# pennneutrinos/chroma

Measured on AMD Instinct MI355X. Metric: photons/sec (propagate_hit), higher is better.
Workload: dtype f32

## Files before the change

### chroma_amd/csrc/chroma_hip.hip

```cpp
#include <math.h>
#include <stdio.h>
#include <stdlib.h>
#include <string.h>
#include <algorithm>

#ifndef CHROMA_EXPERIMENTAL
#define CHROMA_EXPERIMENTAL 0
#endif
#ifndef CHROMA_HYBRID_RENDER
#define CHROMA_HYBRID_RENDER 1
#endif
#include "chroma_internal.h"
#include "propagate_device.h"

#include "kernel_propagate_fused.h"

#include "kernel_step_control.h"

#include "kernels_raycast_crosscheck.h"

#include "kernel_raycast_quad.h"

#include "kernel_raycast_pair.h"

// ... 175 lines not shown
    std::vector<Slab> slabs;
};

static void tracks_release(chroma_ctx *ctx, chroma_tracks *tr)
{
    if (!tr) return;
    for (const chroma_tracks::Slab &s : tr->slabs) chroma_free(ctx, s.rows);
    chroma_free(ctx, tr->rows0);
    chroma_free(ctx, tr->offsets);
    delete tr;
}

namespace { struct PropagateCall; }
static int propagate_order(PropagateCall &call, uint32_t **d_order);

namespace {
struct PropagateCall {
    const CallScope &scope; CallState &cs;
    chroma_ctx *ctx; chroma_geometry *geom;
    CallPlan plan;
    PhotonView pv; chroma_rng rng; chroma_propagate_options opt;
    uint64_t nphotons; uint32_t ncopies;
    uint32_t *in_q, *out_q;
    float4 *work_in, *work_out;
    float4 *rays, *rays_next;
    float4 *final_rec;
    uint32_t final_epoch;
    HitsOut ho;
    bool finalize;
    chroma_propagate_stats acc;
    long long n_upper;
    bool finalized;
    chroma_tracks *tracks;

    hipEvent_t *events(int step) const { return opt.time_kernels ? cs.step_events.data() + EV_PER_STEP * step : nullptr; }

    int load_working()
    {
        const unsigned blocks = (unsigned)std::min<uint64_t>((nphotons + PHYS_BLOCK - 1) / PHYS_BLOCK, (uint64_t)ctx->physics_blocks);
        int rc = scope.clear_words(W_PACKET_USE, W_PACKET_END - W_PACKET_USE); if (rc) return rc;
        uint32_t *d_order = nullptr;
        rc = propagate_order(*this, &d_order); if (rc) return rc;
        hipLaunchKernelGGL(k_load_working, dim3(blocks), dim3(PHYS_BLOCK), 0, ctx->stream, geom->view, pv, in_q, work_in,
                           (uint64_t)nphotons, ncopies, (uint32_t)(nphotons / ncopies), plan.chain ? rays : nullptr,
                           plan.packet == 2 ? cs.d_words + W_PACKET_COHERENT : nullptr, (const uint32_t *)d_order, plan.cast == Cast::LITERAL ? 1 : 0);
        if (d_order) { chroma_free(ctx, d_order); acc.reordered += nphotons; }
#if CHROMA_EXPERIMENTAL
        if (plan.packet)
            hipLaunchKernelGGL(k_packet_decide, dim3(1), dim3(1), 0, ctx->stream, cs.d_words + W_PACKET_COHERENT, cs.d_words + W_PACKET_USE,
                               (uint64_t)nphotons, plan.packet);
#endif
        HIP_TRY(hipGetLastError());
        return CHROMA_OK;
    }

    void launch_step_begin(uint32_t first_n)
    {
        hipLaunchKernelGGL(k_step_begin, dim3(1), dim3(1), 0, ctx->stream, in_q, out_q, cs.d_step,
                           tracks ? 0u : opt.use_weights ? 0xFFFFFFFFu : (uint32_t)(PROP_BLOCK * 16 * 8), first_n);
    }

    void launch_physics(int scatter_first, int fixup)
    {
        StepState *st = cs.d_step;
        float4 *chained = plan.chain ? rays_next : nullptr;
        const bool plain = geom->view.plain_optics != 0;
        bool deal = false;
#if PHYS_DEAL
        deal = plain && !final_rec;
#endif
        const int pb = deal ? PHYS_DEAL_BLOCK : PHYS_BLOCK_OF(!plain);
        unsigned blocks = (unsigned)std::min<long long>((n_upper + pb - 1) / pb, std::max<long long>(1, (long long)ctx->physics_blocks * PHYS_BLOCK / pb));
        if (fixup == 1 && plain) blocks = std::max(std::min(blocks, 64u), blocks / 8);
        DeviceCounters *pc = plan.counting ? cs.d_counters : nullptr;
#if PHYS_DEAL
        if (deal) {
            hipLaunchKernelGGL(k_physics_deal, dim3(blocks), dim3(PHYS_DEAL_BLOCK), 0, ctx->stream, geom->view, pv, st, work_in, out_q, work_out,
                               cs.hit_triangle, cs.hit_distance, rng.seed, rng.photon_id_base, opt.use_weights, scatter_first,
                               cs.retry_list, fixup, pc, chained);
            return;
        }
#endif
        const int literal_rays = fixup == 2 ? 1 : 0;
        with_bool(!plain, [&](auto FULL) {
            hipLaunchKernelGGL((k_physics<FULL>), dim3(blocks), dim3(PHYS_BLOCK_OF(FULL)), 0, ctx->stream, geom->view, pv, st, work_in, out_q,
                               work_out, cs.hit_triangle, cs.hit_distance, rng.seed, rng.photon_id_base, opt.use_weights, scatter_first,
                               cs.retry_list, fixup, pc, chained, final_rec, final_epoch, literal_rays);
        });
    }

    int launch_split_step(int scatter_first, hipEvent_t *ev, uint32_t first_n, bool packet)
    {
        if (n_upper <= 0) return CHROMA_OK;
        StepState *st = cs.d_step;
        const Cast cast = plan.cast;
        const bool exact = cast == Cast::LITERAL || cast == Cast::LITERAL_LANE;
        const dim3 block(PROP_BLOCK);
        auto record = [&](int slot) { return ev ? hipEventRecord(ev[slot], ctx->stream) : hipSuccess; };
        const unsigned rblocks = (unsigned)std::min<long long>((n_upper + PROP_BLOCK - 1) / PROP_BLOCK, 8 * 256);
        auto retry = [&](auto C) {
            hipLaunchKernelGGL((k_raycast_retry<C>), dim3(rblocks), block, 0, ctx->stream, geom->view, rays, st, cs.hit_triangle,
                               cs.hit_distance, cs.retry_list, cs.d_counters);
        };
        launch_step_begin(first_n);
        HIP_TRY(record(EV_STEP_BEGIN));
        if (!plan.chain) {
            unsigned sblocks = (unsigned)std::min<long long>((n_upper + 255) / 256, (long long)ctx->physics_blocks * 4);
            hipLaunchKernelGGL(k_ray_setup, dim3(sblocks), dim3(256), 0, ctx->stream, geom->view, work_in, st, rays,
                               cs.hit_triangle, cs.hit_distance, cs.retry_list, &st->retry, cast == Cast::LITERAL ? 1 : 0);
        }
        HIP_TRY(record(EV_PACKET_BEGIN));
        const uint32_t *skip_quad = nullptr;
#if CHROMA_EXPERIMENTAL
        if (packet) {
            skip_quad = cs.d_words + W_PACKET_USE;
            const unsigned pwaves = (unsigned)std::min<long long>((n_upper + WAVE - 1) / WAVE, (long long)ctx->waves[(int)Cast::QUAD]);
            with_bool(plan.counting, [&](auto C) {
                hipLaunchKernelGGL((k_raycast_packet<C>), dim3(pwaves), block, 0, ctx->stream, geom->view, rays, st, cs.hit_triangle,
                                   cs.hit_distance, cs.retry_list, cs.d_counters, cs.d_words + W_PACKET_USE);
            });
        }
#else
        (void)packet;
#endif
        HIP_TRY(record(EV_CAST_BEGIN));
        const dim3 grid(cast_waves(ctx, cast, n_upper));
        const int chained = plan.chain ? 1 : 0;
        with_bool(plan.counting, [&](auto C) {
            switch (cast) {
            case Cast::PAIR:
                hipLaunchKernelGGL((k_raycast_pair<C>), grid, block, 0, ctx->stream, geom->view, rays, 0, st, cs.hit_triangle,
                                   cs.hit_distance, cs.retry_list, cs.coop_spill, cs.d_counters, ctx->coop_chunk);
                break;
            case Cast::QUAD:
                hipLaunchKernelGGL((k_raycast_quad<C>), grid, block, 0, ctx->stream, geom->view, rays, 0, st, cs.hit_triangle,
                                   cs.hit_distance, cs.retry_list, cs.coop_spill, cs.d_counters, ctx->coop_chunk, chained, skip_quad,
                                   ctx->claim_static);
                break;
            case Cast::COOP:
                hipLaunchKernelGGL((k_raycast_coop<C>), grid, block, 0, ctx->stream, geom->view, rays, 0, st, cs.hit_triangle,
                                   cs.hit_distance, cs.retry_list, cs.coop_spill, cs.d_counters, ctx->coop_chunk);
                break;
            case Cast::WIDE:
                hipLaunchKernelGGL((k_raycast_wide<C>), grid, block, 0, ctx->stream, geom->view, rays, 0, st, cs.hit_triangle,
                                   cs.hit_distance, cs.retry_list, cs.wide_spill, cs.d_counters, ctx->ray_chunk);
                break;
            case Cast::PERSISTENT:
                hipLaunchKernelGGL((k_raycast_persistent<C>), grid, block, 0, ctx->stream, geom->view, rays, 0, st, cs.hit_triangle,
                                   cs.hit_distance, cs.retry_list, cs.d_counters);
                break;
            case Cast::LITERAL:
                hipLaunchKernelGGL((k_raycast_literal<C>), grid, block, 0, ctx->stream, geom->view, rays, st, cs.hit_triangle,
                                   cs.hit_distance, cs.coop_spill, cs.d_counters, ctx->coop_chunk, chained, cs.retry_list,
                                   ctx->claim_static);
                retry(C);
                break;
            case Cast::LITERAL_LANE:
                hipLaunchKernelGGL((k_raycast_retry<C, true>), grid, block, 0, ctx->stream, geom->view, rays, st, cs.hit_triangle,
                                   cs.hit_distance, cs.retry_list, cs.d_counters);
                break;
            }
        });
        HIP_TRY(record(EV_CAST_END));
        launch_physics(scatter_first, exact ? 2 : 0);
        HIP_TRY(record(EV_PHYSICS_END));
        if (!exact) {
            with_bool(plan.counting, retry);
            launch_physics(scatter_first, 1);
        }
        HIP_TRY(record(EV_STEP_END));
// ... 756 lines not shown
```

### chroma_amd/csrc/chroma_internal.h

```cpp
#pragma once
#include <hip/hip_runtime.h>
#include <stdint.h>
#include <array>
#include <map>
#include <mutex>
#include <type_traits>
#include <unordered_map>
#include <vector>

#include <rccl/rccl.h>

#include "device_common.h"

#define CHROMA_LOCAL __attribute__((visibility("hidden")))

CHROMA_LOCAL int set_error(int code, const char *fmt, ...);

#define HIP_TRY(expr)                                                                          \
    do {                                                                                       \
        hipError_t e_ = (expr);                                                                \
        if (e_ != hipSuccess)                                                                  \
            return set_error((int)e_, "%s failed: %s (%s:%d)", #expr, hipGetErrorString(e_), __FILE__, __LINE__); \
    } while (0)

struct CallState {
    uint32_t *queue_a = nullptr, *queue_b = nullptr;
    size_t queue_capacity = 0;
    int32_t *hit_triangle = nullptr;
    float *hit_distance = nullptr;
    uint32_t *retry_list = nullptr;
    float4 *rays = nullptr;
    float4 *rays_b = nullptr;
    float4 *work_a = nullptr, *work_b = nullptr;
    float4 *final_rec = nullptr; size_t final_capacity = 0; uint32_t final_epoch = 0;
    DeviceCounters *d_counters = nullptr;
    uint32_t *d_words = nullptr;
    uint32_t *h_words = nullptr;
    StepState *d_step = nullptr;
    uint32_t *h_step = nullptr;
    std::vector<hipEvent_t> step_events;
    uint2 *wide_spill = nullptr;
    uint2 *coop_spill = nullptr;
    hipEvent_t ev_start = nullptr, ev_stop = nullptr, ev_mid = nullptr;
    hipStream_t aux_stream = nullptr;
    void *call_scratch = nullptr; size_t call_scratch_bytes = 0;
    bool particles_have = false; const void *particles_block = nullptr; size_t particles_block_bytes = 0;
    chroma_particle_arrays particles_run = {}; int32_t particles_max_steps = 0;
    hipEvent_t ev_fork = nullptr, ev_join = nullptr;
    int counting = 0;
    int tail_mode = CHROMA_TAIL_COOP;
    int autosort_mode = 0;
    int packet_mode = 0;
    int walk = CHROMA_WALK_QUAD;
};

struct chroma_ctx {
    int device;
    hipStream_t stream;
    int physics_blocks = 256 * 8;
    int waves[CHROMA_WALK_LITERAL_LANE + 1] = {};
    int ray_chunk = 256, coop_chunk = 64;
    int claim_static = 5 | 8 << 4;
    ncclComm_t comm = nullptr;
    int comm_nranks = 1, comm_rank = 0;
    uint32_t *gather_buf = nullptr;
    size_t gather_capacity = 0;
    struct PoolBlock { void *ptr; hipEvent_t ev; };
    std::mutex pool_mu;
    std::multimap<size_t, PoolBlock> pool;
    std::unordered_map<void *, size_t> live;
    std::vector<hipEvent_t> pool_events;
    size_t pool_bytes = 0, pool_limit = 0;
    uint64_t pool_hits = 0, pool_misses = 0;
    hipStream_t copy_stream = nullptr;
    std::mutex stage_mu;
    static constexpr int STAGE_N = 3;
    static constexpr size_t STAGE_BYTES = 64u << 20;
    void *stage[STAGE_N] = {nullptr, nullptr, nullptr};
    hipEvent_t stage_ev[STAGE_N] = {nullptr, nullptr, nullptr};
    std::mutex stage_down_mu;
    void *stage_down[STAGE_N] = {nullptr, nullptr, nullptr};
    hipEvent_t stage_down_ev[STAGE_N] = {nullptr, nullptr, nullptr};
private:
    friend class CallScope;
    std::mutex call_mu;
    CallState call_state;
};

struct chroma_geometry {
    chroma_ctx *ctx;
    GeoView view;
    std::vector<void *> allocations;
    void *d_vertices = nullptr, *d_triangles = nullptr, *d_material_codes = nullptr, *d_colors = nullptr;
    void *d_nodes_api = nullptr;
    size_t nvertices = 0, ntriangles = 0, nnodes = 0, nwide = 0, nrecords = 0;
    uint32_t stack_need = 0, wide_depth = 0, wide_stack_need = 0;
    size_t device_bytes = 0;
};

enum ScratchWord {
    W_HIT_COUNT = 0,
    W_SURVIVORS = 1,
    W_ABORT = 2,
    W_RESULT_END = 3,
    W_PACKET_USE = 4,
    W_PACKET_COHERENT = 5, W_PACKET_WAVES = 6, W_PACKET_END = 7,
    W_ORDER_PROBE = 8, W_ORDER_PROBE_END = 11,
    SCRATCH_WORDS = 16
};

class CallScope {
public:
    explicit CallScope(chroma_ctx *c) : ctx(c), lock_(c->call_mu) {}
    CallScope(const CallScope &) = delete;
    CallScope &operator=(const CallScope &) = delete;
    CallState &state() const { return ctx->call_state; }

    int clear_words(ScratchWord first, int count = 1) const
    {
        HIP_TRY(hipMemsetAsync(state().d_words + first, 0, count * sizeof(uint32_t), ctx->stream));
        return CHROMA_OK;
    }
    int clear_results() const { return clear_words(W_HIT_COUNT, W_RESULT_END - W_HIT_COUNT); }
    int read_words(ScratchWord first, int count = 1) const { return read_back(first, state().d_words + first, count); }
    int read_results() const { return read_words(W_HIT_COUNT, W_RESULT_END - W_HIT_COUNT); }
    uint32_t word(ScratchWord slot) const { return state().h_words[slot]; }
    int read_word(ScratchWord slot, uint32_t *out) const
    {
        const int rc = read_words(slot);
        *out = word(slot);
        return rc;
    }
    int read_survivors(const uint32_t *d_queue, long long *n) const
    {
        const int rc = read_back(W_SURVIVORS, d_queue, 1);
        *n = (long long)word(W_SURVIVORS) - 1;
        return rc;
    }

    chroma_ctx *const ctx;
private:
    int read_back(ScratchWord slot, const uint32_t *d_src, int count) const
    {
        HIP_TRY(hipMemcpyAsync(state().h_words + slot, d_src, count * sizeof(uint32_t), hipMemcpyDeviceToHost, ctx->stream));
        HIP_TRY(hipStreamSynchronize(ctx->stream));
        return CHROMA_OK;
    }
    std::lock_guard<std::mutex> lock_;
};

struct QueueBuffer { void **ptr; size_t bytes; };
static inline std::array<QueueBuffer, 9> queue_buffers(CallState &c)
{
    return {{{(void **)&c.queue_a, sizeof(uint32_t)}, {(void **)&c.queue_b, sizeof(uint32_t)},
             {(void **)&c.hit_triangle, sizeof(int32_t)}, {(void **)&c.hit_distance, sizeof(float)},
             {(void **)&c.retry_list, sizeof(uint32_t)}, {(void **)&c.rays, 4 * sizeof(float4)}, {(void **)&c.rays_b, 4 * sizeof(float4)},
             {(void **)&c.work_a, 4 * sizeof(float4)}, {(void **)&c.work_b, 4 * sizeof(float4)}}};
}

CHROMA_LOCAL hipError_t ctx_malloc(chroma_ctx *ctx, void **ptr, size_t bytes);

static int grow_call_scratch(const CallScope &scope, size_t need, bool *grew = nullptr)
{
    CallState &cs = scope.state();
    if (grew) *grew = false;
    if (cs.call_scratch_bytes >= need) return CHROMA_OK;
    HIP_TRY(hipStreamSynchronize(scope.ctx->stream));
    if (cs.call_scratch) { HIP_TRY(hipFree(cs.call_scratch)); cs.call_scratch = nullptr; cs.call_scratch_bytes = 0; }
    HIP_TRY(ctx_malloc(scope.ctx, &cs.call_scratch, need));
    cs.call_scratch_bytes = need;
    if (grew) *grew = true;
    return CHROMA_OK;
}

// ... 62 lines not shown
```

### chroma_amd/csrc/device_common.h

```cpp
#pragma once

#include <hip/hip_runtime.h>
#include <stdint.h>

#define CM_FN __host__ __device__ static inline
#include "../../include/chroma_math.h"
#include "../../include/chroma_hip.h"

#define WAVE 64

typedef float f32x2 __attribute__((ext_vector_type(2)));

struct v3 { float x, y, z; };
__device__ inline v3 mk3(float x, float y, float z) { return v3{x, y, z}; }
__device__ inline v3 operator-(v3 a) { return mk3(-a.x, -a.y, -a.z); }
__device__ inline v3 operator+(v3 a, v3 b) { return mk3(a.x + b.x, a.y + b.y, a.z + b.z); }
__device__ inline v3 operator-(v3 a, v3 b) { return mk3(a.x - b.x, a.y - b.y, a.z - b.z); }
__device__ inline v3 operator*(v3 a, float c) { return mk3(a.x * c, a.y * c, a.z * c); }
__device__ inline v3 operator*(float c, v3 a) { return mk3(c * a.x, c * a.y, c * a.z); }
__device__ inline v3 operator/(v3 a, float c) { return mk3(a.x / c, a.y / c, a.z / c); }
__device__ inline v3 operator/(v3 a, v3 b) { return mk3(a.x / b.x, a.y / b.y, a.z / b.z); }
__device__ inline v3 operator/(float c, v3 a) { return mk3(c / a.x, c / a.y, c / a.z); }
__device__ inline float dot(v3 a, v3 b) { return a.x * b.x + a.y * b.y + a.z * b.z; }
__device__ inline v3 cross(v3 a, v3 b)
{ return mk3(a.y * b.z - a.z * b.y, a.z * b.x - a.x * b.z, a.x * b.y - a.y * b.x); }
__device__ inline float norm(v3 a) { return cm_sqrtf(dot(a, a)); }
__device__ inline v3 normalize(v3 a) { return a / norm(a); }

__device__ inline v3 load3(const float *p, size_t i) { return mk3(p[3 * i], p[3 * i + 1], p[3 * i + 2]); }
__device__ inline void store3(float *p, size_t i, v3 v) { p[3 * i] = v.x; p[3 * i + 1] = v.y; p[3 * i + 2] = v.z; }

__device__ inline float interp_table(float x, int n, const float *xp, const float *fp)
{
    int lower = 0;
    int upper = n - 1;
    if (x <= xp[lower]) return fp[lower];
    if (x >= xp[upper]) return fp[upper];
    while (lower < upper - 1) {
        int half = (lower + upper) / 2;
        if (x < xp[half]) upper = half; else lower = half;
    }
    float df = fp[upper] - fp[lower];
    float dx = xp[upper] - xp[lower];
    return fp[lower] + df * (x - xp[lower]) / dx;
}

struct SurfaceInfo { uint32_t model; uint32_t transmissive; float thickness; int32_t dichroic_index; };

#ifndef TRI_STRIDE
#define TRI_STRIDE 3
#endif
struct GeoView {
    const uint4  *nodes;
    const uint4  *wnodes;
    const float4 *tri;
    const float4 *tri_isect;
    const uint4  *tri_phys;
    const uint32_t *tri_to_dev, *dev_to_tri;
    const float *mat_refractive_index, *mat_absorption_length, *mat_scattering_length;
    const uint32_t *mat_num_comp, *mat_comp_offset;
    const float *comp_reemission_prob, *comp_reemission_wvl_cdf, *comp_absorption_length, *comp_reemission_time_cdf;
    const float *surf_detect, *surf_absorb, *surf_reemit, *surf_reflect_diffuse, *surf_reflect_specular,
                *surf_eta, *surf_k, *surf_reemission_cdf;
    const SurfaceInfo *surf_info;
    const uint32_t *dichroic_nangles, *dichroic_offset;
    const float *dichroic_angles, *dichroic_reflect, *dichroic_transmit;
    const uint32_t *solid_id_map;
    const int32_t  *solid_id_to_channel_index;
    float world_origin[3];
    float world_scale;
    float suspect_margin;
    float slab_grow;
    uint32_t wavelength_n; float wavelength_start, wavelength_step;
    uint32_t time_n;       float time_start, time_step;
    uint32_t nnodes, ntriangles, nsolids, nchannels, nwide;
    uint32_t plain_optics;
};

struct TriPhys { v3 normal; uint32_t code, id, bx, by, bz; };
__device__ inline TriPhys load_tri_phys(const GeoView &g, size_t record)
{
    const uint4 *r = g.tri_phys + 2 * record;
    const uint4 a = r[0], b = r[1];
    return TriPhys{mk3(__uint_as_float(a.x), __uint_as_float(a.y), __uint_as_float(a.z)), a.w, b.x, b.y, b.z, b.w};
}

struct PhotonView {
    float *pos, *dir, *pol, *wavelengths, *t;
    uint32_t *flags; int32_t *last_hit_triangles; float *weights; uint32_t *evidx; uint32_t *rng_counters;
};

struct DeviceCounters {
    unsigned long long photon_steps, nodes_visited, triangles_tested, stack_overflows;
    unsigned long long stack_spills;
    unsigned long long packet_rays, packet_nodes, packet_tris;
};

struct StepState {
    uint32_t n;
    uint32_t renorm;
    uint32_t in_tail;
    uint32_t launches;
    uint32_t work;
    uint32_t retry;
    uint32_t pad[2];
};

__device__ inline int hit_channel(const GeoView &g, uint32_t history, int triangle_id, uint32_t detection_state)
{
    if (!(history & detection_state)) return -1;
    if (triangle_id <= -1) return -1;
    uint32_t solid_id = g.solid_id_map[triangle_id];
    return g.solid_id_to_channel_index[solid_id];
}

struct HitsOut {
    PhotonView dst; int32_t *channels; uint32_t capacity;
    uint32_t *hit_count, *earliest;
    uint32_t detection_state; int want;
};

struct Photon {
    v3 position, direction, polarization;
    float wavelength, time, weight;
    uint32_t history;
    int last_hit_triangle;
    uint32_t evidx;
};

CM_FN uint32_t photon_tail_stamp(uint32_t epoch) { return epoch | 0x80000000u; }

struct PhotonRecord {
    float4 row[4];

    PhotonRecord() = default;
    __device__ inline PhotonRecord(const Photon &p, uint32_t draw_counter, int last_hit, uint32_t tag)
    {
        row[0] = make_float4(p.position.x, p.position.y, p.position.z, p.wavelength);
        row[1] = make_float4(p.direction.x, p.direction.y, p.direction.z, p.time);
        row[2] = make_float4(p.polarization.x, p.polarization.y, p.polarization.z, p.weight);
        row[3] = make_float4(__uint_as_float(p.history), __uint_as_float(draw_counter), __int_as_float(last_hit), __uint_as_float(tag));
    }
    __device__ static inline PhotonRecord load(const float4 *r) { PhotonRecord rec; rec.row[0] = r[0]; rec.row[1] = r[1]; rec.row[2] = r[2]; rec.row[3] = r[3]; return rec; }
    __device__ inline void store(float4 *r) const { r[0] = row[0]; r[1] = row[1]; r[2] = row[2]; r[3] = row[3]; }
    __device__ static inline void store_tag(float4 *r, uint32_t tag) { r[3] = make_float4(0.f, 0.f, 0.f, __uint_as_float(tag)); }

    __device__ inline v3 position() const { return mk3(row[0].x, row[0].y, row[0].z); }
    __device__ inline v3 direction() const { return mk3(row[1].x, row[1].y, row[1].z); }
    __device__ inline int last_hit() const { return __float_as_int(row[3].z); }
};

__device__ inline void store_photon(const PhotonView &pv, size_t id, const Photon &p, uint32_t draw_counter)
{
    pv.rng_counters[id] = draw_counter;
    store3(pv.pos, id, p.position);
    store3(pv.dir, id, p.direction);
    store3(pv.pol, id, p.polarization);
    pv.wavelengths[id] = p.wavelength;
    pv.t[id] = p.time;
    pv.flags[id] = p.history;
    pv.last_hit_triangles[id] = p.last_hit_triangle;
    pv.weights[id] = p.weight;
}

__device__ inline void copy_photon(const PhotonView &src, size_t i, const PhotonView &dst, size_t o)
{
    store3(dst.pos, o, load3(src.pos, i));
    store3(dst.dir, o, load3(src.dir, i));
    store3(dst.pol, o, load3(src.pol, i));
    dst.wavelengths[o] = src.wavelengths[i];
    dst.t[o] = src.t[i];
    dst.flags[o] = src.flags[i];
    dst.last_hit_triangles[o] = src.last_hit_triangles[i];
    dst.weights[o] = src.weights[i];
    dst.evidx[o] = src.evidx[i];
    if (dst.rng_counters && src.rng_counters) dst.rng_counters[o] = src.rng_counters[i];
}

#define COPY_ITEMS 16

__device__ inline unsigned lane_id() { return __lane_id(); }

__device__ inline void wave_queue_append(uint32_t *queue, bool pred, uint32_t value)
{
    unsigned long long mask = __ballot(pred);
    if (mask == 0ull) return;
    unsigned lane = lane_id();
    unsigned leader = (unsigned)__ffsll((long long)mask) - 1u;
    uint32_t base = 0;
    if (lane == leader) base = atomicAdd(queue, (uint32_t)__popcll(mask));
    base = __shfl(base, (int)leader);
    if (pred) {
        unsigned rank = (unsigned)__popcll(mask & ((1ull << lane) - 1ull));
        queue[base + rank] = value;
    }
}

template <int MAX_WAVES>
__device__ inline uint32_t block_queue_append(uint32_t *queue, bool pred, uint32_t value, uint32_t *s_counts )
{
    unsigned long long mask = __ballot(pred);
    unsigned lane = lane_id();
    unsigned wave = threadIdx.x / WAVE, nwaves = (blockDim.x + WAVE - 1) / WAVE;
    if (lane == 0) s_counts[wave] = (uint32_t)__popcll(mask);
    __syncthreads();
    if (threadIdx.x == 0) {
        uint32_t total = 0;
        for (unsigned w = 0; w < nwaves; w++) { uint32_t c = s_counts[w]; s_counts[w] = total; total += c; }
        s_counts[MAX_WAVES] = total ? atomicAdd(queue, total) : 0u;
    }
    __syncthreads();
    uint32_t at = 0;
    if (pred) {
        at = s_counts[MAX_WAVES] + s_counts[wave] + (uint32_t)__popcll(mask & ((1ull << lane) - 1ull));
        queue[at] = value;
    }
    return at;
}

__device__ inline unsigned long long wave_sum_u64(unsigned long long v)
{
    for (int off = 32; off > 0; off >>= 1) v += __shfl_down(v, off);
    return v;
}
```

### chroma_amd/csrc/geometry.hip

```cpp
#include <math.h>
#include <stdio.h>
#include <stdlib.h>
#include <string.h>
#include <algorithm>
#include <atomic>
#include <chrono>
#include <string>

#include "chroma_internal.h"
#include "propagate_device.h"
#include "wide_build.h"
#include "host_utils.h"

#include "kernels_geometry.h"

template <class T>
static int upload(chroma_geometry *g, const T *host, size_t count, const T **dev_out)
{
    *dev_out = nullptr;
    size_t bytes = std::max(count, (size_t)1) * sizeof(T);
    void *d = nullptr;
    HIP_TRY(ctx_malloc(g->ctx, &d, bytes));
    g->allocations.push_back(d);
    g->device_bytes += bytes;
// ... 209 lines not shown
        }
        hipFree(d_rank);
        if (rc != CHROMA_OK) { chroma_geometry_destroy(g); return rc; }
        v.tri = (const float4 *)dtri;
    }
    {
        void *dphys = nullptr;
        size_t bytes = std::max<size_t>(nrecords, 1) * 32;
        hipError_t e = ctx_malloc(ctx, &dphys, bytes);
        if (e != hipSuccess) { chroma_geometry_destroy(g); return set_error((int)e, "hipMalloc(%zu) for physics records: %s", bytes, hipGetErrorString(e)); }
        g->allocations.push_back(dphys);
        g->device_bytes += bytes;
        if (nrecords) hipLaunchKernelGGL(k_triangle_phys, dim3((unsigned)((nrecords + 255) / 256)), dim3(256), 0, ctx->stream, v, (uint32_t)nrecords, (uint4 *)dphys);
        e = hipStreamSynchronize(ctx->stream);
        if (e == hipSuccess) e = hipGetLastError();
        if (e != hipSuccess) { chroma_geometry_destroy(g); return set_error((int)e, "physics records: %s", hipGetErrorString(e)); }
        v.tri_phys = (const uint4 *)dphys;
    }
    {
        void *disect = nullptr;
        size_t bytes = std::max<size_t>(nrecords, 1) * 48;
        hipError_t e = ctx_malloc(ctx, &disect, bytes);
        if (e != hipSuccess) { chroma_geometry_destroy(g); return set_error((int)e, "hipMalloc(%zu) for intersection records: %s", bytes, hipGetErrorString(e)); }
        g->allocations.push_back(disect);
        g->device_bytes += bytes;
        if (nrecords) hipLaunchKernelGGL(k_triangle_isect, dim3((unsigned)((nrecords + 255) / 256)), dim3(256), 0, ctx->stream, v, (uint32_t)nrecords, (float4 *)disect);
        e = hipStreamSynchronize(ctx->stream);
        if (e == hipSuccess) e = hipGetLastError();
        if (e != hipSuccess) { chroma_geometry_destroy(g); return set_error((int)e, "intersection records: %s", hipGetErrorString(e)); }
        v.tri_isect = (const float4 *)disect;
    }
    phase("triangle records");
    { const uint32_t *p; if ((rc = upload(g, d->colors, d->colors ? d->ntriangles : 0, &p)) != CHROMA_OK) { chroma_geometry_destroy(g); return rc; } g->d_colors = (void *)p; }
    UP(solid_id_map, d->solid_id_map, d->solid_id_map ? d->ntriangles : 0);
    size_t wn = d->wavelength_n;
    UP(mat_refractive_index, d->mat_refractive_index, d->nmaterials * wn);
    UP(mat_absorption_length, d->mat_absorption_length, d->nmaterials * wn);
    UP(mat_scattering_length, d->mat_scattering_length, d->nmaterials * wn);
    UP(mat_num_comp, d->mat_num_comp, d->nmaterials);
    UP(mat_comp_offset, d->mat_comp_offset, d->nmaterials);
    UP(comp_reemission_prob, d->comp_reemission_prob, d->ncomp_total * wn);
    UP(comp_reemission_wvl_cdf, d->comp_reemission_wvl_cdf, d->ncomp_total * wn);
    UP(comp_absorption_length, d->comp_absorption_length, d->ncomp_total * wn);
    UP(comp_reemission_time_cdf, d->comp_reemission_time_cdf, (size_t)d->ncomp_total * d->time_n);
    UP(surf_detect, d->surf_detect, d->nsurfaces * wn);
    UP(surf_absorb, d->surf_absorb, d->nsurfaces * wn);
    UP(surf_reemit, d->surf_reemit, d->nsurfaces * wn);
    UP(surf_reflect_diffuse, d->surf_reflect_diffuse, d->nsurfaces * wn);
    UP(surf_reflect_specular, d->surf_reflect_specular, d->nsurfaces * wn);
    UP(surf_eta, d->surf_eta, d->nsurfaces * wn);
    UP(surf_k, d->surf_k, d->nsurfaces * wn);
    UP(surf_reemission_cdf, d->surf_reemission_cdf, d->nsurfaces * wn);
    {
        std::vector<SurfaceInfo> info(std::max<uint32_t>(d->nsurfaces, 1));
        for (uint32_t s = 0; s < d->nsurfaces; s++)
            info[s] = SurfaceInfo{d->surf_model[s], d->surf_transmissive[s], d->surf_thickness[s],
                                  d->surf_dichroic_index ? d->surf_dichroic_index[s] : -1};
        UP(surf_info, info.data(), info.size());
    }
    UP(dichroic_nangles, d->dichroic_nangles, d->ndichroic);
    UP(dichroic_offset, d->dichroic_offset, d->ndichroic);
    UP(dichroic_angles, d->dichroic_angles, d->ndichroic_angles_total);
    UP(dichroic_reflect, d->dichroic_reflect, d->ndichroic_angles_total * wn);
    UP(dichroic_transmit, d->dichroic_transmit, d->ndichroic_angles_total * wn);
    UP(solid_id_to_channel_index, d->solid_id_to_channel_index, d->nsolids);
#undef UP
    {
        float maxabs = 0.0f;
        for (int a = 0; a < 3; a++)
            maxabs = std::max(maxabs, std::max(fabsf(d->world_origin[a]), fabsf(d->world_origin[a] + 65535.0f * d->world_scale)));
        v.suspect_margin = 2e-6f * maxabs;
        const double bound = ldexp(1.0, -24) * (10.0 * 65534.0 + 2.0 * (double)maxabs / std::max((double)d->world_scale, 1e-30));
        v.slab_grow = (float)std::min(1.0, std::max(0.25, 4.0 * bound));
        if (const char *e = getenv("CHROMA_SLAB_GROW")) v.slab_grow = (float)std::min(1.0, std::max(0.0625, atof(e)));
    }
    v.wavelength_n = d->wavelength_n; v.wavelength_start = d->wavelength_start; v.wavelength_step = d->wavelength_step;
    v.time_n = d->time_n; v.time_start = d->time_start; v.time_step = d->time_step;
    v.nnodes = d->nnodes; v.ntriangles = d->ntriangles; v.nsolids = d->nsolids; v.nchannels = d->nchannels;
    v.plain_optics = 1u;
    for (uint32_t m = 0; m < d->nmaterials; m++) if (d->mat_num_comp[m]) v.plain_optics = 0u;
    for (uint32_t k = 0; k < d->nsurfaces; k++) if (d->surf_model[k] != CHROMA_SURFACE_DEFAULT) v.plain_optics = 0u;
    if (getenv("CHROMA_FULL_PHYSICS")) v.plain_optics = 0u;

    phase("mesh arrays + tables");
    {
        const uint4 *dn = (const uint4 *)g->d_nodes_api;
        const uint32_t nn = (uint32_t)d->nnodes;
        hipStream_t st = ctx->stream;
        uint32_t need = 0;
        if ((rc = stack_need_fixed_point(ctx, d->nnodes, [&](uint32_t *nd, uint32_t *changed) {
                 hipLaunchKernelGGL(k_stack_need_ref, dim3((nn + 255) / 256), dim3(256), 0, st, dn, nn, nd, changed); }, &need)) != CHROMA_OK) {
            chroma_geometry_destroy(g);
            return rc;
        }
        g->stack_need = std::max<uint32_t>(1, need);
    }
    phase("stack need");
    if (g->stack_need > STACK_LDS + STACK_SCRATCH) {
        uint32_t need = g->stack_need;
        chroma_geometry_destroy(g);
        return set_error(CHROMA_ERR_STACK, "BVH needs %u traversal stack entries, more than the %d supported", need, STACK_LDS + STACK_SCRATCH);
    }
    *out = g;
    return CHROMA_OK;
}

int chroma_geometry_destroy(chroma_geometry *g)
{
    if (!g) return CHROMA_OK;
    hipSetDevice(g->ctx->device);
    hipStreamSynchronize(g->ctx->stream);
    for (void *p : g->allocations) hipFree(p);
    delete g;
    return CHROMA_OK;
}

int chroma_geometry_device_ptr(chroma_geometry *g, const char *name, void **d_ptr, size_t *nbytes)
{
    if (!g || !name || !d_ptr) return set_error(CHROMA_ERR_INVALID, "bad argument");
    std::string n(name);
    size_t bytes = 0; void *p = nullptr;
    if (n == "nodes") { p = g->d_nodes_api; bytes = g->nnodes * 16; }
    else if (n == "vertices") { p = g->d_vertices; bytes = g->nvertices * 12; }
    else if (n == "triangles") { p = g->d_triangles; bytes = g->ntriangles * 12; }
    else if (n == "material_codes") { p = g->d_material_codes; bytes = g->ntriangles * 4; }
    else if (n == "colors") { p = g->d_colors; bytes = g->ntriangles * 4; }
    else if (n == "solid_id_map") { p = (void *)g->view.solid_id_map; bytes = g->ntriangles * 4; }
    else if (n == "solid_id_to_channel_index") { p = (void *)g->view.solid_id_to_channel_index; bytes = (size_t)g->view.nsolids * 4; }
    else if (n == "triangle_records") { p = (void *)g->view.tri; bytes = g->nrecords * (16 * TRI_STRIDE); }
    else if (n == "triangle_phys") { p = (void *)g->view.tri_phys; bytes = g->nrecords * 32; }
    else if (n == "triangle_isect") { p = (void *)g->view.tri_isect; bytes = g->nrecords * 48; }
    else if (n == "wide_nodes") { p = (void *)g->view.wnodes; bytes = g->nwide * 128; }
    else if (n == "tri_to_dev") { p = (void *)g->view.tri_to_dev; bytes = g->ntriangles * 4; }
    else if (n == "dev_to_tri") { p = (void *)g->view.dev_to_tri; bytes = g->nrecords * 4; }
    else return set_error(CHROMA_ERR_INVALID, "unknown geometry array '%s'", name);
    *d_ptr = p;
    if (nbytes) *nbytes = bytes;
    return CHROMA_OK;
}

int chroma_geometry_stack_need(chroma_geometry *g, uint32_t *entries)
{
    if (!g || !entries) return set_error(CHROMA_ERR_INVALID, "bad argument");
    *entries = g->stack_need;
    return CHROMA_OK;
}

}
```

### chroma_amd/csrc/kernel_physics.h

```cpp
#pragma once

#ifndef PHYS_BLOCK
#define PHYS_BLOCK 512
#endif
#ifndef PHYS_WAVES_PER_EU
#define PHYS_WAVES_PER_EU 4
#endif
#ifndef PHYS_SORT
#define PHYS_SORT 1
#endif
#define PHYS_CLASSES 8
#ifndef PHYS_PLAIN_WAVES_PER_EU
#define PHYS_PLAIN_WAVES_PER_EU 5
#endif
#ifndef PHYS_PLAIN_BLOCK
#define PHYS_PLAIN_BLOCK 256
#endif
#define PHYS_BLOCK_OF(FULL) ((FULL) ? PHYS_BLOCK : PHYS_PLAIN_BLOCK)
template <bool FULL>
__global__ __launch_bounds__(PHYS_BLOCK_OF(FULL)) __attribute__((amdgpu_waves_per_eu(FULL ? PHYS_WAVES_PER_EU : PHYS_PLAIN_WAVES_PER_EU))) void
k_physics(GeoView g, PhotonView pv, StepState *st, const float4 *work_in, uint32_t *output_queue, float4 *work_out,
          const int32_t *hit_triangle, const float *hit_distance, uint64_t seed, uint64_t id_base,
          int use_weights, int scatter_first, uint32_t *retry_list, int fixup, DeviceCounters *counters, float4 *rays_next,
          float4 *final_rec = nullptr, uint32_t epoch = 0u, int literal_rays = 0)
{
    constexpr int BLOCK = PHYS_BLOCK_OF(FULL);
    __shared__ uint32_t s_counts[BLOCK / WAVE + 1];
    constexpr bool SORT = FULL && (PHYS_SORT != 0);
    __shared__ uint32_t s_class_count[SORT ? BLOCK / WAVE : 1][PHYS_CLASSES];
    __shared__ int32_t s_perm[SORT ? BLOCK : 1];
    const int nthreads = fixup == 1 ? (int)st->retry : (int)st->n, renorm = (int)st->renorm, renorm_next = st->in_tail ? 0 : 1;
    unsigned long long nsteps = 0;
    for (int block_base = blockIdx.x * BLOCK; block_base < nthreads; block_base += gridDim.x * BLOCK) {
    int id = block_base + threadIdx.x;
    bool alive = false;
    uint32_t photon_id = 0;
    Photon p;
    uint32_t counter = 0;
    int last_hit_record = -1;
    int sorted_slot = (id < nthreads) ? id : -1;
    if (SORT && !fixup) {
        uint32_t cls = 0;
        if (id < nthreads) {
            const int tri0 = hit_triangle[id];
            if (tri0 >= 0) {
                const uint32_t code = g.tri_phys[2 * (size_t)tri0].w;
                const int surface = convert(0xFF & (code >> 8));
                cls = 1u + (uint32_t)min(surface + 1, PHYS_CLASSES - 2);
            }
        }
        const unsigned lane = lane_id(), wave = threadIdx.x / WAVE;
        uint32_t my_rank = 0;
#pragma unroll
        for (uint32_t c = 0; c < PHYS_CLASSES; c++) {
            const unsigned long long m = __ballot(cls == c);
            if (cls == c) my_rank = (uint32_t)__popcll(m & ((1ull << lane) - 1ull));
            if (lane == 0) s_class_count[wave][c] = (uint32_t)__popcll(m);
        }
        __syncthreads();
        static_assert(!SORT || PHYS_CLASSES * (BLOCK / WAVE) == WAVE, "one lane per (class, wave) pair");
        if (wave == 0) {
            const uint32_t c = lane / (BLOCK / WAVE), w = lane % (BLOCK / WAVE);
            const uint32_t k = s_class_count[w][c];
            uint32_t incl = k;
            for (int off = 1; off < WAVE; off <<= 1) { const uint32_t v = __shfl_up(incl, off); if ((int)lane >= off) incl += v; }
            s_class_count[w][c] = incl - k;
        }
        __syncthreads();
        s_perm[s_class_count[wave][cls] + my_rank] = (id < nthreads) ? id : -1;
        __syncthreads();
        sorted_slot = s_perm[threadIdx.x];
        __syncthreads();
    }
    if (sorted_slot >= 0) {
        const int slot = fixup == 1 ? (int)retry_list[sorted_slot] : sorted_slot;
        const float4 *w = work_in + 4 * (size_t)slot;
        const float4 w0 = w[0], w1 = w[1], w2 = w[2], w3 = w[3];
        int tri = hit_triangle[slot];
        const float hit_dist = hit_distance[slot];
        TriPhys rec = {};
        if (tri != HIT_RETRY) {
            photon_id = __float_as_uint(w3.w);
            p.position = mk3(w0.x, w0.y, w0.z);
            p.direction = mk3(w1.x, w1.y, w1.z);
            p.polarization = mk3(w2.x, w2.y, w2.z);
            if (renorm) {
                p.direction = p.direction / norm(p.direction);
                p.polarization = p.polarization / norm(p.polarization);
            }
            if (tri >= 0) rec = load_tri_phys(g, (size_t)tri);
            if (!fixup && tri >= 0) {
                const bool regular = FULL ? phys_hit_is_regular(g, rec, p.position, p.direction, hit_dist)
                                          : phys_hit_is_plainly_regular(g, rec, p.position, p.direction, hit_dist);
                if (!regular) {
                    retry_list[atomicAdd(&st->retry, 1u)] = (uint32_t)slot;
                    tri = HIT_RETRY;
                }
            }
        }
        if (tri != HIT_RETRY) {
            if (tri != HIT_NAN) nsteps++;
            p.wavelength = w0.w;
            p.time = w1.w;
            p.weight = w2.w;
            p.history = __float_as_uint(w3.x);
            p.last_hit_triangle = -1;
            p.evidx = 0;
            last_hit_record = __float_as_int(w3.z);
            cm_rng rng;
            cm_rng_init(&rng, seed, id_base + photon_id, __float_as_uint(w3.y));
            if (tri == HIT_NAN) {
                p.last_hit_triangle = last_hit_record >= 0 ? (int)g.dev_to_tri[last_hit_record] : -1;
                p.history |= CHROMA_NO_HIT | CHROMA_NAN_ABORT;
            } else {
                State s;
                if (tri >= 0) apply_hit_phys(s, p, g, rec, hit_dist);
                else apply_hit_dev(s, p, g, tri, hit_dist);
                if (tri != -1) step_after_hit<FULL>(p, s, rng, g, use_weights != 0, scatter_first);
                last_hit_record = (p.last_hit_triangle < 0) ? -1 : tri;
            }
            counter = rng.counter;
            alive = (p.history & CHROMA_TERMINAL_MASK) == 0;
            if (!alive) {
                if (final_rec) {
                    float4 *f = final_rec + 4 * (size_t)photon_id;
                    f[0] = make_float4(p.position.x, p.position.y, p.position.z, p.wavelength);
                    f[1] = make_float4(p.direction.x, p.direction.y, p.direction.z, p.time);
                    f[2] = make_float4(p.polarization.x, p.polarization.y, p.polarization.z, p.weight);
                    f[3] = make_float4(__uint_as_float(p.history), __uint_as_float(counter), __int_as_float(p.last_hit_triangle), __uint_as_float(epoch));
                } else {
                    store_photon(pv, photon_id, p, counter);
                }
            }
        }
    }
    const uint32_t at = block_queue_append<BLOCK / WAVE>(output_queue, alive, photon_id, s_counts);
    if (alive) {
        float4 *w = work_out + 4 * (size_t)(at - 1u);
        w[0] = make_float4(p.position.x, p.position.y, p.position.z, p.wavelength);
        w[1] = make_float4(p.direction.x, p.direction.y, p.direction.z, p.time);
        w[2] = make_float4(p.polarization.x, p.polarization.y, p.polarization.z, p.weight);
        w[3] = make_float4(__uint_as_float(p.history), __uint_as_float(counter), __int_as_float(last_hit_record), __uint_as_float(photon_id));
        if (rays_next) make_ray_record(g, rays_next + 4 * (size_t)(at - 1u), p.position, p.direction, renorm_next, last_hit_record, literal_rays != 0);
    }
    __syncthreads();
    }
    if (counters) {
        nsteps = wave_sum_u64(nsteps);
        if (lane_id() == 0 && nsteps) atomicAdd(&counters->photon_steps, nsteps);
    }
}
```

### chroma_amd/csrc/propagate_device.h

```cpp
#pragma once
#include "device_common.h"
#include <float.h>

#define WEIGHT_LOWER_THRESHOLD 0.0001f
#define CHROMA_EPSILON 1e-6
enum { CMD_BREAK = 0, CMD_CONTINUE = 1, CMD_PASS = 2 };

struct State {
    v3 surface_normal;
    float refractive_index1, refractive_index2;
    float absorption_length, scattering_length;
    int material1;
    int surface_index;
    float distance_to_boundary;
};

struct LaneCounters { uint32_t steps, nodes, tris, overflows, spills; };
enum { FLUSH_STEPS = 1, FLUSH_SPILLS = 2, FLUSH_OVERFLOWS = 4 };
template <bool COUNT, int ALSO = 0>
__device__ inline void flush_counters(const LaneCounters &cnt, DeviceCounters *counters, unsigned lane)
{
    unsigned long long ov = 0;
    if (ALSO & FLUSH_OVERFLOWS) ov = wave_sum_u64(cnt.overflows);
    if (COUNT) {
        const unsigned long long nd = wave_sum_u64(cnt.nodes), tr = wave_sum_u64(cnt.tris);
        const unsigned long long st = (ALSO & FLUSH_STEPS) ? wave_sum_u64(cnt.steps) : 0ull, sx = (ALSO & FLUSH_SPILLS) ? wave_sum_u64(cnt.spills) : 0ull;
        if (lane == 0) {
            if (ALSO & FLUSH_STEPS) atomicAdd(&counters->photon_steps, st);
            atomicAdd(&counters->nodes_visited, nd);
            atomicAdd(&counters->triangles_tested, tr);
            if (sx) atomicAdd(&counters->stack_spills, sx);
        }
    }
    if (lane == 0 && ov) atomicAdd(&counters->stack_overflows, ov);
}

__device__ inline float interp_property(const GeoView &g, float x, const float *fp)
{
    float start = g.wavelength_start, step = g.wavelength_step;
    uint32_t n = g.wavelength_n;
    if (x < start) return fp[0];
    if (x > (start + (float)(n - 1) * step)) return fp[n - 1];
    int jl = cm_f2i((x - start) / step);
    int ju = (jl + 1 < (int)n) ? jl + 1 : (int)n - 1;
    return fp[jl] + (x - (start + (float)jl * step)) * (fp[ju] - fp[jl]) / step;
}
__device__ inline const float *row(const float *tab, const GeoView &g, int idx) { return tab + (size_t)idx * g.wavelength_n; }

#define MT_NEG_EPS  __uint_as_float(0xB58637BDu)
#define MT_ONE_EPS  __uint_as_float(0x3F800008u)
#define MT_POS_EPS  __uint_as_float(0x358637BDu)
__device__ inline bool intersect_triangle(v3 origin, v3 direction, v3 v0, v3 v1, v3 v2, float &distance)
{
    v3 edge1 = v1 - v0;
    v3 edge2 = v2 - v0;
    v3 h = cross(direction, edge2);
    float a = dot(edge1, h);
    if (a > -FLT_EPSILON && a < FLT_EPSILON) return false;
    float f = 1.0f / a;
    v3 s = origin - v0;
    float u = f * dot(s, h);
    if (u < MT_NEG_EPS || u > MT_ONE_EPS) return false;
    v3 q = cross(s, edge1);
    float v = f * dot(direction, q);
    if (v < MT_NEG_EPS || (u + v) > MT_ONE_EPS) return false;
    float t = f * dot(edge2, q);
    if (t > MT_POS_EPS && t < cm_inff()) {
        distance = t;
        return true;
    }
    return false;
}

__device__ inline bool intersect_triangle_edges(f32x2 rx, f32x2 ry, f32x2 rz, const float4 *rec, float &distance, uint32_t &rank)
{
    const float4 w0 = rec[0], w1 = rec[1], w2 = rec[2];
    const f32x2 ex = {w0.x, w0.y}, ey = {w0.z, w0.w}, ez = {w1.x, w1.y};
    const f32x2 sx = {rx.x - w1.z, rx.y}, sy = {ry.x - w1.w, ry.y}, sz = {rz.x - w2.x, rz.y};
    rank = __float_as_uint(w2.y);
    const f32x2 qx = sy * ez - sz * ey, qy = sz * ex - sx * ez, qz = sx * ey - sy * ex;
    const f32x2 at = (ex * qx.yx + ey * qy.yx) + ez * qz.yx;
    const f32x2 uv = (sx * qx.yx + sy * qy.yx) + sz * qz.yx;
    const float a = at.x;
    const float f = 1.0f / a;
    const f32x2 w = (f32x2){f, f} * uv;
    const float u = w.x, v = w.y, t = f * at.y;
    const bool hit = !(a > -FLT_EPSILON && a < FLT_EPSILON) & !(u < MT_NEG_EPS || u > MT_ONE_EPS) &
                     !(v < MT_NEG_EPS || (u + v) > MT_ONE_EPS) & (t > MT_POS_EPS && t < cm_inff());
    distance = t;
    return hit;
}
__device__ inline bool intersect_triangle_edges(v3 origin, v3 direction, const float4 *rec, float &distance)
{
    uint32_t rank;
    float t;
    const bool hit = intersect_triangle_edges((f32x2){origin.x, direction.x}, (f32x2){origin.y, direction.y},
                                              (f32x2){origin.z, direction.z}, rec, t, rank);
    if (hit) distance = t;
    return hit;
}

__device__ inline float box_tmin(v3 origin, v3 noid, v3 inv_dir, v3 lower, v3 upper, float ws)
{
    float tmin = 0.0f, tmax = cm_inff();
    float t0, t1;
    if (cm_isfinite(inv_dir.x)) {
        t0 = lower.x * inv_dir.x + noid.x;
        t1 = upper.x * inv_dir.x + noid.x;
        tmin = cm_fmaxf(tmin, cm_fminf(t0, t1));
        tmax = cm_fminf(tmax, cm_fmaxf(t0, t1));
    } else if (origin.x < lower.x - ws || origin.x > upper.x + ws) return -1.0f;
    if (cm_isfinite(inv_dir.y)) {
        t0 = lower.y * inv_dir.y + noid.y;
        t1 = upper.y * inv_dir.y + noid.y;
        tmin = cm_fmaxf(tmin, cm_fminf(t0, t1));
        tmax = cm_fminf(tmax, cm_fmaxf(t0, t1));
    } else if (origin.y < lower.y - ws || origin.y > upper.y + ws) return -1.0f;
    if (cm_isfinite(inv_dir.z)) {
        t0 = lower.z * inv_dir.z + noid.z;
        t1 = upper.z * inv_dir.z + noid.z;
        tmin = cm_fmaxf(tmin, cm_fminf(t0, t1));
        tmax = cm_fminf(tmax, cm_fmaxf(t0, t1));
    } else if (origin.z < lower.z - ws || origin.z > upper.z + ws) return -1.0f;
    if (tmin > tmax) return -1.0f;
    return tmin;
}

__device__ inline bool reference_tests_leaf(const GeoView &g, uint32_t bx, uint32_t by, uint32_t bz, v3 origin, v3 direction, float t)
// ... 830 lines not shown
```

Before: 908.1 million.

## Pass physics kernel args via struct and device GeoView, use global address-space loads

The physics kernel now takes a single PhysicsArgs struct, with GeoView read through a constant-address-space pointer to a device-uploaded copy instead of passed by value. Rarely used arguments (retry_list, output PhotonView, counters) are re-read lazily from the kernarg segment to cut SGPR/VGPR pressure. Loads and stores are tagged as global address space to avoid flat addressing. The kernel also reuses the precomputed normalized direction from the ray record when available instead of renormalizing. This adds an extra ray load per photon and a geometry upload, and depends on the ray record's w flag meaning what the new code assumes.

```diff
diff --git a/chroma_amd/csrc/chroma_hip.hip b/chroma_amd/csrc/chroma_hip.hip
--- a/chroma_amd/csrc/chroma_hip.hip
+++ b/chroma_amd/csrc/chroma_hip.hip
@@ -281,10 +281,10 @@
         }
 #endif
         const int literal_rays = fixup == 2 ? 1 : 0;
+        const PhysicsArgs args = {pv, (const CHROMA_CONSTANT_AS GeoView *)geom->d_view, st, work_in, rays, out_q, work_out, cs.hit_triangle, cs.hit_distance, rng.seed, rng.photon_id_base,
+                                  opt.use_weights, scatter_first, cs.retry_list, fixup, pc, chained, final_rec, final_epoch, literal_rays};
         with_bool(!plain, [&](auto FULL) {
-            hipLaunchKernelGGL((k_physics<FULL>), dim3(blocks), dim3(PHYS_BLOCK_OF(FULL)), 0, ctx->stream, geom->view, pv, st, work_in, out_q,
-                               work_out, cs.hit_triangle, cs.hit_distance, rng.seed, rng.photon_id_base, opt.use_weights, scatter_first,
-                               cs.retry_list, fixup, pc, chained, final_rec, final_epoch, literal_rays);
+            hipLaunchKernelGGL((k_physics<FULL>), dim3(blocks), dim3(PHYS_BLOCK_OF(FULL)), 0, ctx->stream, args);
         });
     }
 
diff --git a/chroma_amd/csrc/chroma_internal.h b/chroma_amd/csrc/chroma_internal.h
--- a/chroma_amd/csrc/chroma_internal.h
+++ b/chroma_amd/csrc/chroma_internal.h
@@ -90,6 +90,7 @@
 struct chroma_geometry {
     chroma_ctx *ctx;
     GeoView view;
+    const GeoView *d_view = nullptr;
     std::vector<void *> allocations;
     void *d_vertices = nullptr, *d_triangles = nullptr, *d_material_codes = nullptr, *d_colors = nullptr;
     void *d_nodes_api = nullptr;
diff --git a/chroma_amd/csrc/device_common.h b/chroma_amd/csrc/device_common.h
--- a/chroma_amd/csrc/device_common.h
+++ b/chroma_amd/csrc/device_common.h
@@ -29,6 +29,14 @@
 
 __device__ inline v3 load3(const float *p, size_t i) { return mk3(p[3 * i], p[3 * i + 1], p[3 * i + 2]); }
 __device__ inline void store3(float *p, size_t i, v3 v) { p[3 * i] = v.x; p[3 * i + 1] = v.y; p[3 * i + 2] = v.z; }
+
+#define CHROMA_GLOBAL_AS __attribute__((address_space(1)))
+#define CHROMA_CONSTANT_AS __attribute__((address_space(4)))
+typedef uint32_t u32x4_t __attribute__((ext_vector_type(4)));
+template <class T> __device__ inline T load_global(const T *p) { return *(const CHROMA_GLOBAL_AS T *)p; }
+__device__ inline uint4 load_global(const uint4 *p) { const u32x4_t v = *(const CHROMA_GLOBAL_AS u32x4_t *)p; return make_uint4(v.x, v.y, v.z, v.w); }
+template <class T> __device__ inline void store_global(T *p, T v) { *(CHROMA_GLOBAL_AS T *)p = v; }
+__device__ inline void store3_global(float *p, size_t i, v3 v) { store_global(p + 3 * i, v.x); store_global(p + 3 * i + 1, v.y); store_global(p + 3 * i + 2, v.z); }
 
 __device__ inline float interp_table(float x, int n, const float *xp, const float *fp)
 {
@@ -81,7 +89,7 @@
 __device__ inline TriPhys load_tri_phys(const GeoView &g, size_t record)
 {
     const uint4 *r = g.tri_phys + 2 * record;
-    const uint4 a = r[0], b = r[1];
+    const uint4 a = load_global(r), b = load_global(r + 1);
     return TriPhys{mk3(__uint_as_float(a.x), __uint_as_float(a.y), __uint_as_float(a.z)), a.w, b.x, b.y, b.z, b.w};
 }
 
@@ -152,15 +160,15 @@
 
 __device__ inline void store_photon(const PhotonView &pv, size_t id, const Photon &p, uint32_t draw_counter)
 {
-    pv.rng_counters[id] = draw_counter;
-    store3(pv.pos, id, p.position);
-    store3(pv.dir, id, p.direction);
-    store3(pv.pol, id, p.polarization);
-    pv.wavelengths[id] = p.wavelength;
-    pv.t[id] = p.time;
-    pv.flags[id] = p.history;
-    pv.last_hit_triangles[id] = p.last_hit_triangle;
-    pv.weights[id] = p.weight;
+    store_global(pv.rng_counters + id, draw_counter);
+    store3_global(pv.pos, id, p.position);
+    store3_global(pv.dir, id, p.direction);
+    store3_global(pv.pol, id, p.polarization);
+    store_global(pv.wavelengths + id, p.wavelength);
+    store_global(pv.t + id, p.time);
+    store_global(pv.flags + id, p.history);
+    store_global(pv.last_hit_triangles + id, p.last_hit_triangle);
+    store_global(pv.weights + id, p.weight);
 }
 
 __device__ inline void copy_photon(const PhotonView &src, size_t i, const PhotonView &dst, size_t o)
diff --git a/chroma_amd/csrc/geometry.hip b/chroma_amd/csrc/geometry.hip
--- a/chroma_amd/csrc/geometry.hip
+++ b/chroma_amd/csrc/geometry.hip
@@ -315,6 +315,8 @@
     for (uint32_t k = 0; k < d->nsurfaces; k++) if (d->surf_model[k] != CHROMA_SURFACE_DEFAULT) v.plain_optics = 0u;
     if (getenv("CHROMA_FULL_PHYSICS")) v.plain_optics = 0u;
 
+    if ((rc = upload(g, (const GeoView *)&v, 1, &g->d_view)) != CHROMA_OK) { chroma_geometry_destroy(g); return rc; }
+
     phase("mesh arrays + tables");
     {
         const uint4 *dn = (const uint4 *)g->d_nodes_api;
diff --git a/chroma_amd/csrc/kernel_physics.h b/chroma_amd/csrc/kernel_physics.h
--- a/chroma_amd/csrc/kernel_physics.h
+++ b/chroma_amd/csrc/kernel_physics.h
@@ -17,13 +17,39 @@
 #define PHYS_PLAIN_BLOCK 256
 #endif
 #define PHYS_BLOCK_OF(FULL) ((FULL) ? PHYS_BLOCK : PHYS_PLAIN_BLOCK)
+struct PhysicsArgs {
+    PhotonView pv;
+    const CHROMA_CONSTANT_AS GeoView *geo;
+    StepState *st;
+    const float4 *work_in, *rays; uint32_t *output_queue; float4 *work_out;
+    const int32_t *hit_triangle; const float *hit_distance;
+    uint64_t seed, id_base;
+    int use_weights, scatter_first;
+    uint32_t *retry_list; int fixup;
+    DeviceCounters *counters;
+    float4 *rays_next, *final_rec; uint32_t epoch; int literal_rays;
+};
+__device__ inline const CHROMA_CONSTANT_AS PhysicsArgs *physics_args_in_memory()
+{
+    const CHROMA_CONSTANT_AS PhysicsArgs *a = (const CHROMA_CONSTANT_AS PhysicsArgs *)__builtin_amdgcn_kernarg_segment_ptr();
+    asm volatile("" : "+s"(a));
+    return a;
+}
+
 template <bool FULL>
 __global__ __launch_bounds__(PHYS_BLOCK_OF(FULL)) __attribute__((amdgpu_waves_per_eu(FULL ? PHYS_WAVES_PER_EU : PHYS_PLAIN_WAVES_PER_EU))) void
-k_physics(GeoView g, PhotonView pv, StepState *st, const float4 *work_in, uint32_t *output_queue, float4 *work_out,
-          const int32_t *hit_triangle, const float *hit_distance, uint64_t seed, uint64_t id_base,
-          int use_weights, int scatter_first, uint32_t *retry_list, int fixup, DeviceCounters *counters, float4 *rays_next,
-          float4 *final_rec = nullptr, uint32_t epoch = 0u, int literal_rays = 0)
+k_physics(PhysicsArgs args)
 {
+    const GeoView &g = *(const GeoView *)args.geo;
+    StepState *const st = args.st;
+    const float4 *const work_in = args.work_in, *const rays = args.rays;
+    uint32_t *const output_queue = args.output_queue;
+    float4 *const work_out = args.work_out, *const rays_next = args.rays_next, *const final_rec = args.final_rec;
+    const int32_t *const hit_triangle = args.hit_triangle;
+    const float *const hit_distance = args.hit_distance;
+    const uint64_t seed = args.seed, id_base = args.id_base;
+    const int use_weights = args.use_weights, scatter_first = args.scatter_first, fixup = args.fixup, literal_rays = args.literal_rays;
+    const uint32_t epoch = args.epoch;
     constexpr int BLOCK = PHYS_BLOCK_OF(FULL);
     __shared__ uint32_t s_counts[BLOCK / WAVE + 1];
     constexpr bool SORT = FULL && (PHYS_SORT != 0);
@@ -44,7 +70,7 @@
         if (id < nthreads) {
             const int tri0 = hit_triangle[id];
             if (tri0 >= 0) {
-                const uint32_t code = g.tri_phys[2 * (size_t)tri0].w;
+                const uint32_t code = load_global((const uint32_t *)(g.tri_phys + 2 * (size_t)tri0) + 3);
                 const int surface = convert(0xFF & (code >> 8));
                 cls = 1u + (uint32_t)min(surface + 1, PHYS_CLASSES - 2);
             }
@@ -73,11 +99,13 @@
         __syncthreads();
     }
     if (sorted_slot >= 0) {
-        const int slot = fixup == 1 ? (int)retry_list[sorted_slot] : sorted_slot;
+        const int slot = fixup == 1 ? (int)load_global(physics_args_in_memory()->retry_list + sorted_slot) : sorted_slot;
         const float4 *w = work_in + 4 * (size_t)slot;
         const float4 w0 = w[0], w1 = w[1], w2 = w[2], w3 = w[3];
         int tri = hit_triangle[slot];
         const float hit_dist = hit_distance[slot];
+        float4 ray1 = make_float4(0.f, 0.f, 0.f, __int_as_float(HIT_RETRY));
+        if (renorm) ray1 = rays[4 * (size_t)slot + 1];
         TriPhys rec = {};
         if (tri != HIT_RETRY) {
             photon_id = __float_as_uint(w3.w);
@@ -85,7 +113,8 @@
             p.direction = mk3(w1.x, w1.y, w1.z);
             p.polarization = mk3(w2.x, w2.y, w2.z);
             if (renorm) {
-                p.direction = p.direction / norm(p.direction);
+                if (__float_as_int(ray1.w) == 0) p.direction = mk3(ray1.x, ray1.y, ray1.z);
+                else p.direction = p.direction / norm(p.direction);
                 p.polarization = p.polarization / norm(p.polarization);
             }
             if (tri >= 0) rec = load_tri_phys(g, (size_t)tri);
@@ -93,7 +122,7 @@
                 const bool regular = FULL ? phys_hit_is_regular(g, rec, p.position, p.direction, hit_dist)
                                           : phys_hit_is_plainly_regular(g, rec, p.position, p.direction, hit_dist);
                 if (!regular) {
-                    retry_list[atomicAdd(&st->retry, 1u)] = (uint32_t)slot;
+                    store_global(physics_args_in_memory()->retry_list + atomicAdd(&st->retry, 1u), (uint32_t)slot);
                     tri = HIT_RETRY;
                 }
             }
@@ -110,7 +139,7 @@
             cm_rng rng;
             cm_rng_init(&rng, seed, id_base + photon_id, __float_as_uint(w3.y));
             if (tri == HIT_NAN) {
-                p.last_hit_triangle = last_hit_record >= 0 ? (int)g.dev_to_tri[last_hit_record] : -1;
+                p.last_hit_triangle = last_hit_record >= 0 ? (int)load_global(g.dev_to_tri + last_hit_record) : -1;
                 p.history |= CHROMA_NO_HIT | CHROMA_NAN_ABORT;
             } else {
                 State s;
@@ -129,7 +158,10 @@
                     f[2] = make_float4(p.polarization.x, p.polarization.y, p.polarization.z, p.weight);
                     f[3] = make_float4(__uint_as_float(p.history), __uint_as_float(counter), __int_as_float(p.last_hit_triangle), __uint_as_float(epoch));
                 } else {
-                    store_photon(pv, photon_id, p, counter);
+                    const CHROMA_CONSTANT_AS PhotonView *late = &physics_args_in_memory()->pv;
+                    const PhotonView out = {late->pos, late->dir, late->pol, late->wavelengths, late->t, late->flags, late->last_hit_triangles,
+                                            late->weights, late->evidx, late->rng_counters};
+                    store_photon(out, photon_id, p, counter);
                 }
             }
         }
@@ -145,7 +177,7 @@
     }
     __syncthreads();
     }
-    if (counters) {
+    if (DeviceCounters *counters = physics_args_in_memory()->counters) {
         nsteps = wave_sum_u64(nsteps);
         if (lane_id() == 0 && nsteps) atomicAdd(&counters->photon_steps, nsteps);
     }
diff --git a/chroma_amd/csrc/propagate_device.h b/chroma_amd/csrc/propagate_device.h
--- a/chroma_amd/csrc/propagate_device.h
+++ b/chroma_amd/csrc/propagate_device.h
@@ -39,11 +39,12 @@
 {
     float start = g.wavelength_start, step = g.wavelength_step;
     uint32_t n = g.wavelength_n;
-    if (x < start) return fp[0];
-    if (x > (start + (float)(n - 1) * step)) return fp[n - 1];
+    if (x < start) return load_global(fp);
+    if (x > (start + (float)(n - 1) * step)) return load_global(fp + (n - 1));
     int jl = cm_f2i((x - start) / step);
     int ju = (jl + 1 < (int)n) ? jl + 1 : (int)n - 1;
-    return fp[jl] + (x - (start + (float)jl * step)) * (fp[ju] - fp[jl]) / step;
+    const float lo = load_global(fp + jl);
+    return lo + (x - (start + (float)jl * step)) * (load_global(fp + ju) - lo) / step;
 }
 __device__ inline const float *row(const float *tab, const GeoView &g, int idx) { return tab + (size_t)idx * g.wavelength_n; }
 
```

Measured after the change: 915.5 million (median of 6 runs). About the same (+0.8%).
